# ToddThomson/Mila

Measured on AMD Instinct MI355X. Metric: Gemma-4 12B decode tok/s (B=1, context 2048), 1xMI355X, higher is better.
Workload: dtype bf16; 1 GPU; Gemma-4 12B, weight policy bf16, B=1, prefill T=2048 then decode at positions 2048..; decode_mode=graph, replicas=1, parallelism=replicas only (no collective), bounded_local_kv=0

## Files before the change

mila_amd/csrc/matvec.hip:

```cpp
#include <cstdio>
#include <cstdlib>

#include "common.h"
#include "internal.h"
#include "rms_common.h"
#include "matvec_body.h"

namespace mila {

struct MatvecTail
{
    void* y;
    const float* scales;
    const uint16_t* bias;
    const uint16_t* post_w;
    uint16_t* res_out;
    float post_scale, eps;
    int group, comb_splits, comb_heads;
    float* amax_v;
    int* amax_i;
};
static MatvecTail matvec_tail(const MatvecParams& p)
{
    return MatvecTail{p.y, p.scales, p.bias, p.post_w, p.res_out, p.post_scale, p.eps, p.group, p.comb_splits, p.comb_heads, p.amax_v, p.amax_i};
}

template <int FMT, int R, int U, int PRO, bool GEGLU, bool F32OUT, int XC, int XSRC = X_PLAIN>
__global__ __launch_bounds__(1024) void matvec_kernel(const uint8_t* W, const uint16_t* x, const uint16_t* norm_w, const uint16_t* res, int K, int N, int nblocks,
                                                      const MatvecTail t)
{
    extern __shared__ __attribute__((aligned(16))) unsigned char smem_raw[];
    __shared__ float red_a[16 * XC], red_b[16 * XC];
    u32x4 rkeep[XC];
    const MatvecParams p{t.y, x, W, t.scales, t.bias, norm_w, t.post_w, res, t.res_out, t.post_scale, t.eps, K, N, t.group, t.comb_splits, t.comb_heads, t.amax_v, t.amax_i};
    matvec_body<FMT, R, U, PRO, GEGLU, F32OUT ? Y_F32 : Y_BF16, XC, XSRC, RES_MEM>(
        p, reinterpret_cast<u32x4*>(smem_raw), red_a, red_b, (int)blockIdx.x, nblocks, rkeep, NoWait{});
}

static int g_tune_R = 0, g_tune_U = 0, g_tune_blocks = 0;
MILA_TUNE("matvec.rows_per_wave", g_tune_R);
MILA_TUNE("matvec.chunks_in_flight", g_tune_U);
MILA_TUNE("matvec.max_workgroups", g_tune_blocks);
static thread_local int t_last_matvec_blocks = 0;

template <int FMT, int R, int U, int PRO, bool GEGLU, bool F32OUT, int XC>
static int launch_xc(const MatvecParams& p, int max_blocks, hipStream_t s)
{
    const int n_rg = (p.N + R - 1) / R;
    constexpr int EPC = Fmt<FMT>::kElemsPerChunk;
    const int nchunks = p.K / EPC;
    const int S = (nchunks + 64 * U - 1) / (64 * U);
    const size_t lds = (size_t)S * 64 * U * EPC * 2;
    MILA_REQUIRE(lds <= 65536, "matvec: K=%d needs %zu bytes of LDS for x (limit 65536)", p.K, lds);
    int blocks = (n_rg + kMatvecWaves - 1) / kMatvecWaves;
    if (blocks > max_blocks) blocks = max_blocks;
    if (blocks < 1) blocks = 1;
    t_last_matvec_blocks = blocks;
    note_form("matvec");
    hipLaunchKernelGGL((matvec_kernel<FMT, R, U, PRO, GEGLU, F32OUT, XC>), dim3(blocks), dim3(64 * kMatvecWaves), lds, s, p.W, p.x, p.norm_w, p.res, p.K, p.N, blocks,
                       matvec_tail(p));
    MILA_LAUNCH_CHECK("matvec");
}

template <int FMT, int R, int U, int PRO, bool GEGLU, bool F32OUT>
static int launch(const MatvecParams& p, int max_blocks, hipStream_t s)
{
    if (p.K <= 8192) return launch_xc<FMT, R, U, PRO, GEGLU, F32OUT, 1>(p, max_blocks, s);
    if (p.K <= 16384) return launch_xc<FMT, R, U, PRO, GEGLU, F32OUT, 2>(p, max_blocks, s);
    return set_error(MILA_E_INVALID_ARGUMENT, "matvec: K=%d exceeds the register-staged x limit (16384)", p.K);
}

struct ShapeOverrides
{
    struct E { bool set = false; int rows = 1, U = 2, blocks = kNumCU; } e[3][3];
};
static ShapeOverrides parse_shape_overrides()
{
    ShapeOverrides o;
    const char* env = getenv("MILA_MATVEC_SHAPE");
    if (!env) return o;
    int f, t, r, u, b, n = 0;
    while (*env && sscanf(env, "f%dt%d=%d,%d,%d%n", &f, &t, &r, &u, &b, &n) == 5)
    {
        if (f >= 0 && f < 3 && t >= 0 && t < 3 && r >= 1 && u >= 1 && b >= 1) { o.e[f][t].set = true; o.e[f][t].rows = r; o.e[f][t].U = u; o.e[f][t].blocks = b; }
        env += n;
        if (*env == ';') ++env;
    }
    return o;
}

MatvecShape matvec_launch_shape(int fmt, bool geglu, int N, bool argmax)
{
    const int rows = geglu ? 2 * N : N;
    const bool tall = rows >= 16384, huge = rows >= 100000;
    int rows_per_step, U;
    if (fmt == FMT_BF16) { rows_per_step = huge ? 4 : (tall ? 2 : 1); U = tall ? 2 : 4; }
    else if (fmt == FMT_FP8) { rows_per_step = huge ? 4 : (tall ? 2 : 1); U = 2; }
    else { rows_per_step = tall ? 2 : 1; U = huge ? 2 : 1; }
    int max_blocks = (huge || (tall && fmt == FMT_BF16)) ? 2 * kNumCU : kNumCU;
    {
        static const ShapeOverrides ov = parse_shape_overrides();
        const ShapeOverrides::E& e = ov.e[fmt][huge ? 2 : (tall ? 1 : 0)];
        if (e.set) { rows_per_step = e.rows; U = e.U; max_blocks = e.blocks; }
    }
    int R = geglu ? (rows_per_step >= 2 ? rows_per_step / 2 : 1) : rows_per_step;
    if (g_tune_R > 0) R = g_tune_R;
    if (g_tune_U > 0) U = g_tune_U;
    if (g_tune_blocks > 0) max_blocks = g_tune_blocks;
    if (argmax && max_blocks > kArgmaxPartials) max_blocks = kArgmaxPartials;
    if (geglu && R > 2) R = 2;
    if (R == 1) U = (U == 1 || U == 2) ? U : 4;
    else if (R == 2) U = (U == 1) ? 1 : 2;
    else { R = geglu ? 2 : 4; U = 2; }
    return MatvecShape{R, U, max_blocks};
}

template <int FMT, int PRO, bool GEGLU, bool F32OUT>
static int dispatch_RU(const MatvecParams& p, hipStream_t s)
{
    const MatvecShape shape = matvec_launch_shape(FMT, GEGLU, p.N, p.amax_v != nullptr);
    const int R = shape.R, U = shape.U, max_blocks = shape.max_blocks;
    if (R == 1 && U == 1) return launch<FMT, 1, 1, PRO, GEGLU, F32OUT>(p, max_blocks, s);
    if (R == 1 && U == 2) return launch<FMT, 1, 2, PRO, GEGLU, F32OUT>(p, max_blocks, s);
    if (R == 1) return launch<FMT, 1, 4, PRO, GEGLU, F32OUT>(p, max_blocks, s);
    if (R == 2 && U == 1) return launch<FMT, 2, 1, PRO, GEGLU, F32OUT>(p, max_blocks, s);
    if (R == 2) return launch<FMT, 2, 2, PRO, GEGLU, F32OUT>(p, max_blocks, s);
    if constexpr (!GEGLU) return launch<FMT, 4, 2, PRO, GEGLU, F32OUT>(p, max_blocks, s);
    return launch<FMT, 2, 2, PRO, GEGLU, F32OUT>(p, max_blocks, s);
}

template <int FMT, int U, int XSRC>
static int launch_combine_t(const MatvecParams& p, hipStream_t s)
{
    constexpr int EPC = Fmt<FMT>::kElemsPerChunk;
    const int nchunks = p.K / EPC;
    const int S = (nchunks + 64 * U - 1) / (64 * U);
    const size_t lds = (size_t)S * 64 * U * EPC * 2;
    MILA_REQUIRE(lds <= 65536, "matvec_attn_combine: K=%d needs %zu bytes of LDS for x (limit 65536)", p.K, lds);
    int blocks = (p.N + kMatvecWaves - 1) / kMatvecWaves;
    if (blocks > kNumCU) blocks = kNumCU;
    hipLaunchKernelGGL((matvec_kernel<FMT, 1, U, 0, false, false, 1, XSRC>), dim3(blocks), dim3(64 * kMatvecWaves), lds, s, p.W, p.x, p.norm_w, p.res, p.K, p.N, blocks,
                       matvec_tail(p));
    MILA_LAUNCH_CHECK("matvec_attn_combine");
}
template <int XSRC>
static int launch_combine(int fmt, const MatvecParams& p, hipStream_t s)
{
    switch (fmt)
    {
        case FMT_BF16: return launch_combine_t<FMT_BF16, 4, XSRC>(p, s);
        case FMT_FP8: return launch_combine_t<FMT_FP8, 2, XSRC>(p, s);
        default: return launch_combine_t<FMT_FP4, 1, XSRC>(p, s);
    }
}

static int validate(const char* who, const void* y, const void* x, const void* W, const float* scales,
                    int fmt, int K, int N, int group)
{
    MILA_REQUIRE(y && x && W, "%s: null pointer (y=%p x=%p W=%p)", who, y, x, W);
    MILA_REQUIRE(K > 0 && N > 0, "%s: K and N must be positive (K=%d N=%d)", who, K, N);
    MILA_REQUIRE(K <= 16384, "%s: K=%d exceeds the register-staged x limit (16384)", who, K);
    if (fmt == FMT_BF16) MILA_REQUIRE(K % 8 == 0, "%s: K=%d must be a multiple of 8 for bf16 weights", who, K);
    if (fmt == FMT_FP8)
    {
        MILA_REQUIRE(K % 16 == 0, "%s: K=%d must be a multiple of 16 for fp8 weights", who, K);
        MILA_REQUIRE(scales != nullptr, "%s: fp8 weights need per-channel scales", who);
    }
    if (fmt == FMT_FP4)
    {
        MILA_REQUIRE(group == 64 || group == 128, "%s: fp4 group size must be 64 or 128 (got %d)", who, group);
        MILA_REQUIRE(K % 32 == 0 && K % group == 0, "%s: K=%d must be a multiple of 32 and of the group size %d", who, K, group);
        MILA_REQUIRE(scales != nullptr, "%s: fp4 weights need per-group scales", who);
    }
    MILA_REQUIRE(fmt >= 0 && fmt <= 2, "%s: unknown weight format %d", who, fmt);
    return MILA_OK;
}

template <int PRO, bool GEGLU, bool F32OUT>
static int dispatch_fmt(int fmt, const MatvecParams& p, hipStream_t s)
{
    switch (fmt)
    {
        case FMT_BF16: return dispatch_RU<FMT_BF16, PRO, GEGLU, F32OUT>(p, s);
        case FMT_FP8: return dispatch_RU<FMT_FP8, PRO, GEGLU, F32OUT>(p, s);
        default: return dispatch_RU<FMT_FP4, PRO, GEGLU, F32OUT>(p, s);
    }
}

}

using namespace mila;

extern "C" {

int mila_cdna4_matvec_bf16(uint16_t* y, const uint16_t* x, const uint16_t* W, const uint16_t* bias, int K,
                           int N, mila_stream_t stream)
{
    int rc = validate("matvec_bf16", y, x, W, nullptr, FMT_BF16, K, N, 0);
    if (rc) return rc;
    MatvecParams p{y, x, reinterpret_cast<const uint8_t*>(W), nullptr, bias, nullptr, nullptr, nullptr, nullptr, 1.0f, 0.0f, K, N, 0, 0, 0};
    return dispatch_fmt<0, false, false>(FMT_BF16, p, as_stream(stream));
}

int mila_cdna4_matvec_bf16_qfp8(uint16_t* y, const uint16_t* x, const uint8_t* W, const float* scales,
                                const uint16_t* bias, int K, int N, mila_stream_t stream)
{
    int rc = validate("matvec_bf16_qfp8", y, x, W, scales, FMT_FP8, K, N, 0);
    if (rc) return rc;
    MatvecParams p{y, x, W, scales, bias, nullptr, nullptr, nullptr, nullptr, 1.0f, 0.0f, K, N, 0, 0, 0};
    return dispatch_fmt<0, false, false>(FMT_FP8, p, as_stream(stream));
}

int mila_cdna4_matvec_bf16_qfp4(uint16_t* y, const uint16_t* x, const uint8_t* W_packed, const float* scales,
                                const uint16_t* bias, int K, int N, int group, mila_stream_t stream)
{
    int rc = validate("matvec_bf16_qfp4", y, x, W_packed, scales, FMT_FP4, K, N, group);
    if (rc) return rc;
    MatvecParams p{y, x, W_packed, scales, bias, nullptr, nullptr, nullptr, nullptr, 1.0f, 0.0f, K, N, group, 0, 0};
    return dispatch_fmt<0, false, false>(FMT_FP4, p, as_stream(stream));
}

int mila_cdna4_matvec_f32out(float* y, const uint16_t* x, const void* W, const float* scales, int fmt, int K,
                             int N, int group, mila_stream_t stream)
{
    int rc = validate("matvec_f32out", y, x, W, scales, fmt, K, N, group);
    if (rc) return rc;
    MatvecParams p{y, x, reinterpret_cast<const uint8_t*>(W), scales, nullptr, nullptr, nullptr, nullptr, nullptr, 1.0f, 0.0f, K, N, group, 0, 0};
    return dispatch_fmt<0, false, true>(fmt, p, as_stream(stream));
}

int mila_cdna4_matvec_attn_combine(uint16_t* y, const void* partials, int splits, int NH, int HS, const void* W, const float* scales,
                                   int fmt, int N, int group, mila_stream_t stream)
{
    MILA_REQUIRE(partials != nullptr, "matvec_attn_combine: null partials");
    MILA_REQUIRE(HS == 256 || HS == 512, "matvec_attn_combine: head size %d must be 256 or 512 (a wave's 64 chunks span 2 or 1 heads)", HS);
    MILA_REQUIRE(NH > 0 && splits > 1 && splits <= 64, "matvec_attn_combine: need NH > 0 and 1 < splits <= 64 (NH=%d splits=%d)", NH, splits);
    const int K = NH * HS;
    MILA_REQUIRE(K <= 8192, "matvec_attn_combine: NH * HS = %d exceeds 8192", K);
    int rc = validate("matvec_attn_combine", y, partials, W, scales, fmt, K, N, group);
    if (rc) return rc;
    MatvecParams p{y, reinterpret_cast<const uint16_t*>(partials), reinterpret_cast<const uint8_t*>(W), scales, nullptr, nullptr, nullptr, nullptr,
                   nullptr, 1.0f, 0.0f, K, N, group, splits, NH};
    return HS == 512 ? launch_combine<X_COMBINE_1>(fmt, p, as_stream(stream)) : launch_combine<X_COMBINE_2>(fmt, p, as_stream(stream));
}

int mila_cdna4_fused_norm_matvec(const mila_fused_matvec_args* a, mila_stream_t stream)
{
    MILA_REQUIRE(a != nullptr, "fused_norm_matvec: null args");
    const int rows = a->geglu ? 2 * a->N : a->N;
    (void)rows;
    int rc = validate("fused_norm_matvec", a->y, a->x, a->W, a->scales, a->fmt, a->K, a->N, a->group);
    if (rc) return rc;
    MILA_REQUIRE(a->norm_w != nullptr, "fused_norm_matvec: norm_w is required");
    MILA_REQUIRE((a->res == nullptr) == (a->post_w == nullptr), "fused_norm_matvec: res and post_w go together");
    if (a->res)
    {
        MILA_REQUIRE(a->res_out != nullptr, "fused_norm_matvec: res_out is required with res");
        MILA_REQUIRE(a->res_out != a->res && a->res_out != a->x, "fused_norm_matvec: res_out must not alias res or x");
    }
    MatvecParams p{a->y, a->x, reinterpret_cast<const uint8_t*>(a->W), a->scales, nullptr, a->norm_w, a->post_w,
                   a->res, a->res_out, a->post_scale, a->eps, a->K, a->N, a->group, 0, 0};
    hipStream_t s = as_stream(stream);
    MILA_REQUIRE(!(a->geglu && a->f32_out), "fused_norm_matvec: geglu and f32_out are exclusive");
    if (a->argmax_scratch)
    {
        MILA_REQUIRE(a->f32_out, "fused_norm_matvec: argmax_scratch needs f32_out (the logits)");
        MILA_REQUIRE(a->argmax_blocks != nullptr, "fused_norm_matvec: argmax_blocks is required with argmax_scratch");
        if (a->argmax_scratch_bytes < mila_cdna4_sample_scratch_bytes())
            return set_error(MILA_E_SCRATCH_TOO_SMALL, "fused_norm_matvec: argmax scratch %zu bytes < required %zu", a->argmax_scratch_bytes, mila_cdna4_sample_scratch_bytes());
        p.amax_v = reinterpret_cast<float*>(a->argmax_scratch);
        p.amax_i = reinterpret_cast<int*>(p.amax_v + kArgmaxPartials);
    }
    if (a->f32_out)
    {
        rc = a->res ? dispatch_fmt<2, false, true>(a->fmt, p, s) : dispatch_fmt<1, false, true>(a->fmt, p, s);
        if (rc == MILA_OK && a->argmax_scratch)
        {
            if (t_last_matvec_blocks > kArgmaxPartials) return set_error(MILA_E_RUNTIME, "fused_norm_matvec: %d workgroups exceed the %d sampler partials", t_last_matvec_blocks, kArgmaxPartials);
            *a->argmax_blocks = t_last_matvec_blocks;
        }
        return rc;
    }
    if (a->res)
        return a->geglu ? dispatch_fmt<2, true, false>(a->fmt, p, s) : dispatch_fmt<2, false, false>(a->fmt, p, s);
    return a->geglu ? dispatch_fmt<1, true, false>(a->fmt, p, s) : dispatch_fmt<1, false, false>(a->fmt, p, s);
}

}
```

mila_amd/csrc/matvec_body.h:

```cpp
#pragma once
#include "common.h"
#include "rms_common.h"

namespace mila {

enum { FMT_BF16 = 0, FMT_FP8 = 1, FMT_FP4 = 2 };

template <int FMT> struct Fmt;
template <> struct Fmt<FMT_BF16> { static constexpr int kElemsPerChunk = 8; };
template <> struct Fmt<FMT_FP8> { static constexpr int kElemsPerChunk = 16; };
template <> struct Fmt<FMT_FP4> { static constexpr int kElemsPerChunk = 32; };

template <int FMT>
__device__ __forceinline__ float chunk_dot(const u32x4 w, const u32x4* __restrict__ xs, int c, float acc)
{
    if constexpr (FMT == FMT_BF16)
    {
        const u32x4 xv = xs[c];
#pragma unroll
        for (int d = 0; d < 4; ++d) acc = dot2_bf16(as_bf16x2(w[d]), as_bf16x2(xv[d]), acc);
    }
    else if constexpr (FMT == FMT_FP8)
    {
        const u32x4 x0 = xs[2 * c], x1 = xs[2 * c + 1];
        acc = dot2_bf16(fp8x2_to_bf16x2(w[0], false), as_bf16x2(x0[0]), acc);
        acc = dot2_bf16(fp8x2_to_bf16x2(w[0], true), as_bf16x2(x0[1]), acc);
        acc = dot2_bf16(fp8x2_to_bf16x2(w[1], false), as_bf16x2(x0[2]), acc);
        acc = dot2_bf16(fp8x2_to_bf16x2(w[1], true), as_bf16x2(x0[3]), acc);
        acc = dot2_bf16(fp8x2_to_bf16x2(w[2], false), as_bf16x2(x1[0]), acc);
        acc = dot2_bf16(fp8x2_to_bf16x2(w[2], true), as_bf16x2(x1[1]), acc);
        acc = dot2_bf16(fp8x2_to_bf16x2(w[3], false), as_bf16x2(x1[2]), acc);
        acc = dot2_bf16(fp8x2_to_bf16x2(w[3], true), as_bf16x2(x1[3]), acc);
    }
    else
    {
#pragma unroll
        for (int d = 0; d < 4; ++d)
        {
            const u32x4 xv = xs[4 * c + d];
            acc = dot2_bf16(fp4x2_to_bf16x2<0>(w[d]), as_bf16x2(xv[0]), acc);
            acc = dot2_bf16(fp4x2_to_bf16x2<1>(w[d]), as_bf16x2(xv[1]), acc);
            acc = dot2_bf16(fp4x2_to_bf16x2<2>(w[d]), as_bf16x2(xv[2]), acc);
            acc = dot2_bf16(fp4x2_to_bf16x2<3>(w[d]), as_bf16x2(xv[3]), acc);
        }
    }
    return acc;
}

struct MatvecParams
{
    void* y;
    const uint16_t* x;
    const uint8_t* W;
    const float* scales;
    const uint16_t* bias;
    const uint16_t* norm_w;
    const uint16_t* post_w;
    const uint16_t* res;
    uint16_t* res_out;
    float post_scale, eps;
    int K, N, group;
    int comb_splits, comb_heads;
    float* amax_v = nullptr;
    int* amax_i = nullptr;
};

constexpr int kMatvecWaves = 16;

struct MatvecShape { int R, U, max_blocks; };
MatvecShape matvec_launch_shape(int fmt, bool geglu, int N, bool argmax);

template <int FMT, int U, int NR>
struct WBuf
{
    u32x4 w[U][NR];
    float sc[U][NR];
};

__device__ __forceinline__ uint32_t sload32(const void* p_uniform)
{
    uint32_t v;
    asm volatile("s_load_dword %0, %1, 0x0\n\ts_waitcnt lgkmcnt(0)" : "=s"(v) : "s"(p_uniform) : "memory");
    return v;
}

typedef __attribute__((address_space(1))) uint32_t gu32;
typedef __attribute__((address_space(1))) unsigned long long gu64;
__device__ __forceinline__ gu32* as_global(uint32_t* p) { return (gu32*)p; }
__device__ __forceinline__ const gu32* as_global(const uint32_t* p) { return (const gu32*)p; }
__device__ __forceinline__ gu64* as_global(unsigned long long* p) { return (gu64*)p; }
__device__ __forceinline__ const gu64* as_global(const unsigned long long* p) { return (const gu64*)p; }
__device__ __forceinline__ void handoff_store(uint32_t* v, int i, uint32_t bf16_bits)
{
    __hip_atomic_store(as_global(v) + i, bf16_bits, __ATOMIC_RELAXED, __HIP_MEMORY_SCOPE_AGENT);
}
__device__ __forceinline__ u32x4 handoff_load8(const uint32_t* v, int c)
{
    const gu64* q = as_global(reinterpret_cast<const unsigned long long*>(v)) + (size_t)c * 4;
    u32x4 r;
#pragma unroll
    for (int d = 0; d < 4; ++d)
    {
        const unsigned long long t = __hip_atomic_load(q + d, __ATOMIC_RELAXED, __HIP_MEMORY_SCOPE_AGENT);
        r[d] = ((uint32_t)t & 0xffffu) | ((uint32_t)(t >> 32) << 16);
    }
    return r;
}

struct NoWait { __device__ __forceinline__ void operator()() const {} };

enum { Y_BF16 = 0, Y_F32 = 1, Y_HANDOFF = 2 };
enum { X_PLAIN = 0, X_HANDOFF = 1, X_COMBINE_1 = 2, X_COMBINE_2 = 3 };
enum { RES_MEM = 0, RES_REG = 1 };

template <int FMT, int R, int U, int PRO, bool GEGLU, int YDST, int XC, int XSRC, int RSRC, class Wait>
__device__ __forceinline__ void matvec_body(const MatvecParams& p, u32x4* xs, float* red_a, float* red_b,
                                            const int block, const int nblocks, u32x4 (&rkeep)[XC], Wait wait)
{
    const int tid = threadIdx.x, lane = tid & 63;
    const int wib = __builtin_amdgcn_readfirstlane(tid >> 6);
    const int K = p.K, N = p.N;
    const int nx16 = K / 8;

    constexpr int EPC = Fmt<FMT>::kElemsPerChunk;
    constexpr int XPC = EPC / 8;
    constexpr int NR = GEGLU ? 2 * R : R;
    const int nchunks = K / EPC;
    const size_t row_bytes = (size_t)nchunks * 16;
    const int S = (nchunks + 64 * U - 1) / (64 * U);
    const int nx16_pad = S * 64 * U * XPC;
    const int ngroups = (FMT == FMT_FP4) ? K / p.group : 0;
    const int cpg_shift = (FMT == FMT_FP4) ? (p.group == 128 ? 2 : 1) : 0;
    const int total_waves = nblocks * kMatvecWaves;
    const int n_rg = (N + R - 1) / R;
    const int wave_g = block * kMatvecWaves + wib;
    const int nrg_w = wave_g < n_rg ? (n_rg - 1 - wave_g) / total_waves + 1 : 0;
    const int T = nrg_w * S;

    u32x4 px[XC], pnw[PRO != 0 ? XC : 1], ppw[PRO == 2 ? XC : 1], pres[PRO == 2 ? XC : 1];
#pragma unroll
    for (int k = 0; k < XC; ++k)
    {
        const size_t e = (size_t)min(tid + 1024 * k, nx16 - 1) * 8;
        if constexpr (XSRC == X_PLAIN) px[k] = ld16(p.x + e);
        if constexpr (PRO != 0) pnw[k] = ld16(p.norm_w + e);
        if constexpr (PRO == 2)
        {
            ppw[k] = ld16(p.post_w + e);
            if constexpr (RSRC == RES_MEM) pres[k] = ld16(p.res + e);
            else pres[k] = rkeep[k];
        }
    }

    auto issue = [&](WBuf<FMT, U, NR>& b, int rg, int s) {
        const int c0 = s * (64 * U) + lane;
#pragma unroll
        for (int j = 0; j < NR; ++j)
        {
            const int col = min(rg * R + (GEGLU ? (j >> 1) : j), N - 1);
            const int row = (GEGLU && (j & 1)) ? (N + col) : col;
            const uint8_t* wrow = p.W + (size_t)row * row_bytes;
#pragma unroll
            for (int u = 0; u < U; ++u)
            {
                const int c = min(c0 + 64 * u, nchunks - 1);
                b.w[u][j] = ld16_nt(wrow + (size_t)c * 16);
                if constexpr (FMT == FMT_FP4) b.sc[u][j] = p.scales[(size_t)row * ngroups + (c >> cpg_shift)];
            }
        }
    };
    int ci_rg = wave_g, ci_s = 0, cc_rg = wave_g, cc_s = 0;
    auto advance = [&](int& rg_, int& s_) {
        const bool wrap = (s_ + 1 == S);
        s_ = wrap ? 0 : s_ + 1;
        rg_ = wrap ? rg_ + total_waves : rg_;
    };
    WBuf<FMT, U, NR> ba, bb;
    issue(ba, ci_rg, ci_s); advance(ci_rg, ci_s);
    issue(bb, ci_rg, ci_s); advance(ci_rg, ci_s);

    if constexpr (XSRC == X_COMBINE_1 || XSRC == X_COMBINE_2)
    {
        constexpr int HPW = (XSRC == X_COMBINE_1) ? 1 : 2;
        const float* part = reinterpret_cast<const float*>(p.x);
        const int splits = p.comb_splits, HS = 512 / HPW, STR = HS + 4;
#pragma unroll
        for (int k = 0; k < XC; ++k)
        {
            const int c = tid + 1024 * k;
            const int h0 = ((c & ~63) * 8) / HS;
            const int myj = (HPW == 1) ? 0 : (lane >> 5);
            float fs[HPW], Lh[HPW];
#pragma unroll
            for (int j = 0; j < HPW; ++j)
            {
                const int h = min(h0 + j, p.comb_heads - 1);
                const float* hb = part + (size_t)h * splits * STR;
                const float ms = (lane < splits) ? hb[(size_t)lane * STR + HS] : -INFINITY;
                const float ls = (lane < splits) ? hb[(size_t)lane * STR + HS + 1] : 0.0f;
                const float M = wave_max(ms);
                fs[j] = (ms == -INFINITY) ? 0.0f : __expf(ms - M);
                Lh[j] = wave_sum(ls * fs[j]);
            }
            const int h = min(h0 + myj, p.comb_heads - 1);
            const float* vb = part + (size_t)h * splits * STR + (size_t)((c * 8) % HS);
            float acc[8];
#pragma unroll
            for (int e = 0; e < 8; ++e) acc[e] = 0.0f;
            for (int s0 = 0; s0 < splits; s0 += 8)
            {
                f32x4 va[8], vb2[8];
#pragma unroll
                for (int u = 0; u < 8; ++u)
                {
                    const float* src = vb + (size_t)min(s0 + u, splits - 1) * STR;
                    va[u] = *reinterpret_cast<const f32x4*>(src);
                    vb2[u] = *reinterpret_cast<const f32x4*>(src + 4);
                }
#pragma unroll
                for (int u = 0; u < 8; ++u)
                {
                    const int si = min(s0 + u, 63);
                    float f = __uint_as_float(__builtin_amdgcn_readlane(__float_as_uint(fs[0]), si));
                    if constexpr (HPW == 2)
                    {
                        const float f1 = __uint_as_float(__builtin_amdgcn_readlane(__float_as_uint(fs[1]), si));
                        f = myj ? f1 : f;
                    }
                    if (s0 + u >= splits) f = 0.0f;
#pragma unroll
                    for (int e = 0; e < 4; ++e)
                    {
                        acc[e] = fmaf(va[u][e], f, acc[e]);
                        acc[4 + e] = fmaf(vb2[u][e], f, acc[4 + e]);
                    }
                }
            }
            float L = Lh[0];
            if constexpr (HPW == 2) L = myj ? Lh[1] : Lh[0];
#pragma unroll
            for (int d = 0; d < 4; ++d)
                px[k][d] = pack_bf16x2(L > 0.0f ? acc[2 * d] / L : 0.0f, L > 0.0f ? acc[2 * d + 1] / L : 0.0f);
        }
    }

    wait();
    if constexpr (XSRC == X_HANDOFF)
    {
#pragma unroll
        for (int k = 0; k < XC; ++k)
            px[k] = handoff_load8(reinterpret_cast<const uint32_t*>(p.x), min(tid + 1024 * k, nx16 - 1));
    }

    for (int i = nx16 + tid; i < nx16_pad; i += 1024) xs[i] = u32x4{0u, 0u, 0u, 0u};
    if constexpr (PRO == 0)
    {
#pragma unroll
        for (int k = 0; k < XC; ++k)
            if (tid + 1024 * k < nx16) xs[tid + 1024 * k] = px[k];
    }
    else
    {
        const int G = (nx16 + 63) / 64;
        auto rstd_of = [&](const u32x4* v, float* red) {
#pragma unroll
            for (int k = 0; k < XC; ++k)
            {
                float s = (tid + 1024 * k < nx16) ? sumsq8(v[k], 0.0f) : 0.0f;
                s = wave_sum(s);
                if (lane == 0) red[wib + kMatvecWaves * k] = s;
            }
            __syncthreads();
            float t = 0.0f;
            for (int g = 0; g < G; ++g) t += red[g];
            return rsqrtf(t / (float)K + p.eps);
        };
        if constexpr (PRO == 1)
        {
            const float rstd = rstd_of(px, red_a);
#pragma unroll
            for (int k = 0; k < XC; ++k)
                if (tid + 1024 * k < nx16) xs[tid + 1024 * k] = rms_apply8(px[k], pnw[k], rstd, 0.0f);
        }
        else
        {
            const float rstd_a = rstd_of(px, red_a);
#pragma unroll
            for (int k = 0; k < XC; ++k) rkeep[k] = sandwich_tail8(rms_apply8(px[k], ppw[k], rstd_a, 0.0f), pres[k], p.post_scale);
            if (block == 0 && p.res_out != nullptr)
            {
#pragma unroll
                for (int k = 0; k < XC; ++k)
                    if (tid + 1024 * k < nx16) st16(p.res_out + (size_t)(tid + 1024 * k) * 8, rkeep[k]);
            }
            const float rstd_r = rstd_of(rkeep, red_b);
#pragma unroll
            for (int k = 0; k < XC; ++k)
                if (tid + 1024 * k < nx16) xs[tid + 1024 * k] = rms_apply8(rkeep[k], pnw[k], rstd_r, 0.0f);
        }
    }
    __syncthreads();

    float acc[NR];
#pragma unroll
    for (int j = 0; j < NR; ++j) acc[j] = 0.0f;

    auto compute = [&](const WBuf<FMT, U, NR>& b, int s) {
#pragma unroll
        for (int u = 0; u < U; ++u)
        {
            const int c = s * (64 * U) + lane + 64 * u;
#pragma unroll
            for (int j = 0; j < NR; ++j)
            {
                if constexpr (FMT == FMT_FP4)
                    acc[j] = fmaf(b.sc[u][j], chunk_dot<FMT>(b.w[u][j], xs, c, 0.0f), acc[j]);
                else
                    acc[j] = chunk_dot<FMT>(b.w[u][j], xs, c, acc[j]);
            }
        }
    };

    float amax_bv = -3.402823466e+38f;
    int amax_bi = 0x7fffffff;
    auto finish = [&](int rg_) {
        const int col0 = rg_ * R;
#pragma unroll
        for (int j = 0; j < NR; ++j) acc[j] = wave_sum(acc[j]);
#pragma unroll
        for (int j = 0; j < NR; ++j)
        {
            const int col = min(col0 + (GEGLU ? (j >> 1) : j), N - 1);
            const int row = (GEGLU && (j & 1)) ? (N + col) : col;
            float v = acc[j];
            if constexpr (FMT == FMT_FP8) v = __builtin_bit_cast(float, sload32(p.scales + row)) * v;
            if (p.bias)
            {
                const uint32_t pair = sload32(reinterpret_cast<const uint32_t*>(p.bias) + (row >> 1));
                v += bf16_bits_to_f32((uint16_t)((row & 1) ? (pair >> 16) : (pair & 0xffffu)));
            }
            acc[j] = v;
        }
        if (lane == 0)
        {
#pragma unroll
            for (int r = 0; r < R; ++r)
            {
                const int col = col0 + r;
                if (col >= N) continue;
                float v = acc[r];
                if constexpr (GEGLU)
                {
                    const float g = round_bf16(acc[2 * r]), up = round_bf16(acc[2 * r + 1]);
                    v = gelu_tanh(g) * up;
                }
                if constexpr (YDST == Y_F32)
                {
                    reinterpret_cast<float*>(p.y)[col] = v;
                    if (p.amax_v) argmax_better(amax_bv, amax_bi, v, col);
                }
                else if constexpr (YDST == Y_HANDOFF) handoff_store(reinterpret_cast<uint32_t*>(p.y), col, f32_to_bf16_bits(v));
                else reinterpret_cast<uint16_t*>(p.y)[col] = f32_to_bf16_bits(v);
            }
        }
#pragma unroll
        for (int j = 0; j < NR; ++j) acc[j] = 0.0f;
    };

    auto consume = [&](const WBuf<FMT, U, NR>& b) {
        compute(b, cc_s);
        const int rg_prev = cc_rg;
        advance(cc_rg, cc_s);
        if (cc_rg != rg_prev) finish(rg_prev);
    };

    int t = 0;
    for (; t + 4 <= T; t += 2)
    {
        consume(ba);
        issue(ba, ci_rg, ci_s); advance(ci_rg, ci_s);
        consume(bb);
        issue(bb, ci_rg, ci_s); advance(ci_rg, ci_s);
    }
    const int rem = T - t;
    if (rem >= 1)
    {
        consume(ba);
        if (rem == 3) issue(ba, ci_rg, ci_s);
    }
    if (rem >= 2) consume(bb);
    if (rem == 3) consume(ba);

    if constexpr (YDST == Y_F32)
    {
        if (p.amax_v)
        {
            __syncthreads();
            if (lane == 0) { red_a[wib] = amax_bv; red_b[wib] = __int_as_float(amax_bi); }
            __syncthreads();
            if (tid == 0)
            {
                float bv = red_a[0];
                int bi = __float_as_int(red_b[0]);
#pragma unroll
                for (int w = 1; w < kMatvecWaves; ++w) argmax_better(bv, bi, red_a[w], __float_as_int(red_b[w]));
                p.amax_v[block] = bv;
                p.amax_i[block] = bi;
            }
        }
    }
}

}
```

mila_amd/csrc/matvec_rows.hip:

```cpp
#include <cstdio>

#include "common.h"
#include "internal.h"
#include "rms_common.h"
#include "matvec_body.h"

namespace mila {

constexpr int kMaxMatvecRows = 4;
constexpr size_t kMatvecRowsLdsLimit = 160 * 1024;

struct MatvecRowsTail
{
    void* y;
    const float* scales;
    const uint16_t* bias;
    const uint16_t* post_w;
    uint16_t* res_out;
    float post_scale, eps;
    int group;
    long long x_stride, y_stride, res_stride, res_out_stride;
    float* amax_v;
    long long amax_stride;
};

template <int FMT, int U, int PRO, bool GEGLU, bool F32OUT, int XC, int NB>
__global__ __launch_bounds__(1024) void matvec_rows_kernel(const uint8_t* W, const uint16_t* x, const uint16_t* norm_w, const uint16_t* res, int K, int N, int nblocks,
                                                           const MatvecRowsTail t)
{
    extern __shared__ __attribute__((aligned(16))) unsigned char smem_raw[];
    __shared__ float red[NB][2][16 * XC];
    u32x4* xs0 = reinterpret_cast<u32x4*>(smem_raw);

    const int tid = threadIdx.x, lane = tid & 63;
    const int wib = __builtin_amdgcn_readfirstlane(tid >> 6);
    const int block = (int)blockIdx.x;
    const int nx16 = K / 8;

    constexpr int EPC = Fmt<FMT>::kElemsPerChunk;
    constexpr int XPC = EPC / 8;
    constexpr int NR = GEGLU ? 2 : 1;
    const int nchunks = K / EPC;
    const size_t row_bytes = (size_t)nchunks * 16;
    const int S = (nchunks + 64 * U - 1) / (64 * U);
    const int nx16_pad = S * 64 * U * XPC;
    const int ngroups = (FMT == FMT_FP4) ? K / t.group : 0;
    const int cpg_shift = (FMT == FMT_FP4) ? (t.group == 128 ? 2 : 1) : 0;
    const int total_waves = nblocks * kMatvecWaves;
    const int wave_g = block * kMatvecWaves + wib;
    const int ncol_w = wave_g < N ? (N - 1 - wave_g) / total_waves + 1 : 0;
    const int T = ncol_w * S;

    u32x4 px[NB][XC], pnw[PRO != 0 ? XC : 1], ppw[PRO == 2 ? XC : 1], pres[PRO == 2 ? NB : 1][XC];
#pragma unroll
    for (int k = 0; k < XC; ++k)
    {
        const size_t e = (size_t)min(tid + 1024 * k, nx16 - 1) * 8;
#pragma unroll
        for (int b = 0; b < NB; ++b)
        {
            px[b][k] = ld16(x + (size_t)b * t.x_stride + e);
            if constexpr (PRO == 2) pres[b][k] = ld16(res + (size_t)b * t.res_stride + e);
        }
        if constexpr (PRO != 0) pnw[k] = ld16(norm_w + e);
        if constexpr (PRO == 2) ppw[k] = ld16(t.post_w + e);
    }

    auto issue = [&](WBuf<FMT, U, NR>& wb, int col_, int s) {
        const int c0 = s * (64 * U) + lane;
        const int col = min(col_, N - 1);
#pragma unroll
        for (int j = 0; j < NR; ++j)
        {
            const int row = j ? (N + col) : col;
            const uint8_t* wrow = W + (size_t)row * row_bytes;
#pragma unroll
            for (int u = 0; u < U; ++u)
            {
                const int c = min(c0 + 64 * u, nchunks - 1);
                wb.w[u][j] = ld16_nt(wrow + (size_t)c * 16);
                if constexpr (FMT == FMT_FP4) wb.sc[u][j] = t.scales[(size_t)row * ngroups + (c >> cpg_shift)];
            }
        }
    };
    int ci_col = wave_g, ci_s = 0, cc_col = wave_g, cc_s = 0;
    auto advance = [&](int& col_, int& s_) {
        const bool wrap = (s_ + 1 == S);
        s_ = wrap ? 0 : s_ + 1;
        col_ = wrap ? col_ + total_waves : col_;
    };
    WBuf<FMT, U, NR> ba, bb;
    issue(ba, ci_col, ci_s); advance(ci_col, ci_s);
    issue(bb, ci_col, ci_s); advance(ci_col, ci_s);

#pragma unroll
    for (int b = 0; b < NB; ++b)
        for (int i = nx16 + tid; i < nx16_pad; i += 1024) xs0[(size_t)b * nx16_pad + i] = u32x4{0u, 0u, 0u, 0u};
    if constexpr (PRO == 0)
    {
#pragma unroll
        for (int b = 0; b < NB; ++b)
#pragma unroll
            for (int k = 0; k < XC; ++k)
                if (tid + 1024 * k < nx16) xs0[(size_t)b * nx16_pad + tid + 1024 * k] = px[b][k];
    }
    else
    {
        const int G = (nx16 + 63) / 64;
        auto rstd_of = [&](const u32x4* v, float* r) {
#pragma unroll
            for (int k = 0; k < XC; ++k)
            {
                float s = (tid + 1024 * k < nx16) ? sumsq8(v[k], 0.0f) : 0.0f;
                s = wave_sum(s);
                if (lane == 0) r[wib + kMatvecWaves * k] = s;
            }
            __syncthreads();
            float tt = 0.0f;
            for (int g = 0; g < G; ++g) tt += r[g];
            return rsqrtf(tt / (float)K + t.eps);
        };
#pragma unroll
        for (int b = 0; b < NB; ++b)
        {
            u32x4* xs = xs0 + (size_t)b * nx16_pad;
            if constexpr (PRO == 1)
            {
                const float rstd = rstd_of(px[b], red[b][0]);
#pragma unroll
                for (int k = 0; k < XC; ++k)
                    if (tid + 1024 * k < nx16) xs[tid + 1024 * k] = rms_apply8(px[b][k], pnw[k], rstd, 0.0f);
            }
            else
            {
                u32x4 rk[XC];
                const float rstd_a = rstd_of(px[b], red[b][0]);
#pragma unroll
                for (int k = 0; k < XC; ++k) rk[k] = sandwich_tail8(rms_apply8(px[b][k], ppw[k], rstd_a, 0.0f), pres[b][k], t.post_scale);
                if (block == 0 && t.res_out != nullptr)
                {
#pragma unroll
                    for (int k = 0; k < XC; ++k)
                        if (tid + 1024 * k < nx16) st16(t.res_out + (size_t)b * t.res_out_stride + (size_t)(tid + 1024 * k) * 8, rk[k]);
                }
                const float rstd_r = rstd_of(rk, red[b][1]);
#pragma unroll
                for (int k = 0; k < XC; ++k)
                    if (tid + 1024 * k < nx16) xs[tid + 1024 * k] = rms_apply8(rk[k], pnw[k], rstd_r, 0.0f);
            }
        }
    }
    __syncthreads();

    float acc[NB][NR];
#pragma unroll
    for (int b = 0; b < NB; ++b)
#pragma unroll
        for (int j = 0; j < NR; ++j) acc[b][j] = 0.0f;

    auto compute = [&](const WBuf<FMT, U, NR>& wb, int s) {
#pragma unroll
        for (int u = 0; u < U; ++u)
        {
            const int c = s * (64 * U) + lane + 64 * u;
#pragma unroll
            for (int j = 0; j < NR; ++j)
#pragma unroll
                for (int b = 0; b < NB; ++b)
                {
                    const u32x4* xs = xs0 + (size_t)b * nx16_pad;
                    if constexpr (FMT == FMT_FP4)
                        acc[b][j] = fmaf(wb.sc[u][j], chunk_dot<FMT>(wb.w[u][j], xs, c, 0.0f), acc[b][j]);
                    else
                        acc[b][j] = chunk_dot<FMT>(wb.w[u][j], xs, c, acc[b][j]);
                }
        }
    };

    float amax_bv[NB];
    int amax_bi[NB];
#pragma unroll
    for (int b = 0; b < NB; ++b) { amax_bv[b] = -3.402823466e+38f; amax_bi[b] = 0x7fffffff; }

    auto finish = [&](int col) {
        float scale[NR], bias[NR];
#pragma unroll
        for (int j = 0; j < NR; ++j)
        {
            const int row = j ? (N + col) : col;
            scale[j] = 1.0f;
            bias[j] = 0.0f;
            if constexpr (FMT == FMT_FP8) scale[j] = __builtin_bit_cast(float, sload32(t.scales + row));
            if (t.bias)
            {
                const uint32_t pair = sload32(reinterpret_cast<const uint32_t*>(t.bias) + (row >> 1));
                bias[j] = bf16_bits_to_f32((uint16_t)((row & 1) ? (pair >> 16) : (pair & 0xffffu)));
            }
        }
#pragma unroll
        for (int b = 0; b < NB; ++b)
        {
#pragma unroll
            for (int j = 0; j < NR; ++j)
            {
                float v = wave_sum(acc[b][j]);
                if constexpr (FMT == FMT_FP8) v = scale[j] * v;
                if (t.bias) v += bias[j];
                acc[b][j] = v;
            }
            if (lane == 0)
            {
                float v = acc[b][0];
                if constexpr (GEGLU)
                {
                    const float g = round_bf16(acc[b][0]), up = round_bf16(acc[b][1]);
                    v = gelu_tanh(g) * up;
                }
                if constexpr (F32OUT)
                {
                    reinterpret_cast<float*>(t.y)[(size_t)b * t.y_stride + col] = v;
                    if (t.amax_v) argmax_better(amax_bv[b], amax_bi[b], v, col);
                }
                else reinterpret_cast<uint16_t*>(t.y)[(size_t)b * t.y_stride + col] = f32_to_bf16_bits(v);
            }
#pragma unroll
            for (int j = 0; j < NR; ++j) acc[b][j] = 0.0f;
        }
    };

    auto consume = [&](const WBuf<FMT, U, NR>& wb) {
        compute(wb, cc_s);
        const int col_prev = cc_col;
        advance(cc_col, cc_s);
        if (cc_col != col_prev) finish(col_prev);
    };

    int ts = 0;
    for (; ts + 4 <= T; ts += 2)
    {
        consume(ba);
        issue(ba, ci_col, ci_s); advance(ci_col, ci_s);
        consume(bb);
        issue(bb, ci_col, ci_s); advance(ci_col, ci_s);
    }
    const int rem = T - ts;
    if (rem >= 1)
    {
        consume(ba);
        if (rem == 3) issue(ba, ci_col, ci_s);
    }
    if (rem >= 2) consume(bb);
    if (rem == 3) consume(ba);

    if constexpr (F32OUT)
    {
        if (t.amax_v)
        {
            __syncthreads();
            if (lane == 0)
            {
#pragma unroll
                for (int b = 0; b < NB; ++b) { red[b][0][wib] = amax_bv[b]; red[b][1][wib] = __int_as_float(amax_bi[b]); }
            }
            __syncthreads();
            if (tid < NB)
            {
                float bv = red[tid][0][0];
                int bi = __float_as_int(red[tid][1][0]);
                for (int w = 1; w < kMatvecWaves; ++w) argmax_better(bv, bi, red[tid][0][w], __float_as_int(red[tid][1][w]));
                float* pv = t.amax_v + (size_t)tid * t.amax_stride;
                pv[block] = bv;
                reinterpret_cast<int*>(pv + kArgmaxPartials)[block] = bi;
            }
        }
    }
}

struct MatvecRowsArgs
{
    const uint8_t* W;
    const uint16_t* x;
    const uint16_t* norm_w;
    const uint16_t* res;
    int K, N;
    MatvecRowsTail t;
};

struct MatvecRowsPlan { int R, U, xc; size_t lds, lds_static; int blocks; };

static bool plan_rows(int fmt, int K, int N, bool geglu, bool argmax, int rows, MatvecRowsPlan& pl)
{
    if (fmt < 0 || fmt > 2 || K <= 0 || N <= 0 || K > 16384 || rows < 1 || rows > kMaxMatvecRows) return false;
    const int epc = fmt == FMT_BF16 ? 8 : (fmt == FMT_FP8 ? 16 : 32);
    if (K % epc != 0) return false;
    const MatvecShape shape = matvec_launch_shape(fmt, geglu, N, argmax);
    pl.R = rows == 1 ? shape.R : 1;
    pl.U = shape.U;
    pl.xc = K <= 8192 ? 1 : 2;
    const int nchunks = K / epc;
    const int S = (nchunks + 64 * pl.U - 1) / (64 * pl.U);
    pl.lds = (size_t)rows * S * 64 * pl.U * epc * 2;
    pl.lds_static = rows > 1 ? (size_t)rows * 2 * 16 * pl.xc * sizeof(float) : (size_t)2 * 16 * pl.xc * sizeof(float);
    const int n_rg = (N + pl.R - 1) / pl.R;
    int blocks = (n_rg + kMatvecWaves - 1) / kMatvecWaves;
    if (blocks > shape.max_blocks) blocks = shape.max_blocks;
    pl.blocks = blocks < 1 ? 1 : blocks;
    return true;
}

template <int FMT, int U, int PRO, bool GEGLU, bool F32OUT, int XC, int NB>
static int launch_rows_t(const MatvecRowsArgs& a, const MatvecRowsPlan& pl, hipStream_t s)
{
    auto kernel = matvec_rows_kernel<FMT, U, PRO, GEGLU, F32OUT, XC, NB>;
    static thread_local int raised_for = -1;
    int dev = 0;
    if (pl.lds > 65536)
    {
        int rc = check_hip(hipGetDevice(&dev), "matvec_rows");
        if (rc) return rc;
        if (raised_for != dev)
        {
            rc = check_hip(hipFuncSetAttribute(reinterpret_cast<const void*>(kernel), hipFuncAttributeMaxDynamicSharedMemorySize, (int)kMatvecRowsLdsLimit), "matvec_rows");
            if (rc) return rc;
            raised_for = dev;
        }
    }
    note_form("matvec_rows");
    hipLaunchKernelGGL(kernel, dim3(pl.blocks), dim3(64 * kMatvecWaves), pl.lds, s, a.W, a.x, a.norm_w, a.res, a.K, a.N, pl.blocks, a.t);
    MILA_LAUNCH_CHECK("matvec_rows");
}

template <int FMT, int U, int PRO, bool GEGLU, bool F32OUT, int XC>
static int launch_rows_nb(const MatvecRowsArgs& a, const MatvecRowsPlan& pl, int rows, hipStream_t s)
{
    if (rows == 2) return launch_rows_t<FMT, U, PRO, GEGLU, F32OUT, XC, 2>(a, pl, s);
    if (rows == 3) return launch_rows_t<FMT, U, PRO, GEGLU, F32OUT, XC, 3>(a, pl, s);
    return launch_rows_t<FMT, U, PRO, GEGLU, F32OUT, XC, 4>(a, pl, s);
}

template <int FMT, int PRO, bool GEGLU, bool F32OUT>
static int launch_rows_u(const MatvecRowsArgs& a, const MatvecRowsPlan& pl, int rows, hipStream_t s)
{
    if (pl.xc == 1)
    {
        if (pl.U == 1) return launch_rows_nb<FMT, 1, PRO, GEGLU, F32OUT, 1>(a, pl, rows, s);
        if (pl.U == 2) return launch_rows_nb<FMT, 2, PRO, GEGLU, F32OUT, 1>(a, pl, rows, s);
        return launch_rows_nb<FMT, 4, PRO, GEGLU, F32OUT, 1>(a, pl, rows, s);
    }
    if (pl.U == 1) return launch_rows_nb<FMT, 1, PRO, GEGLU, F32OUT, 2>(a, pl, rows, s);
    if (pl.U == 2) return launch_rows_nb<FMT, 2, PRO, GEGLU, F32OUT, 2>(a, pl, rows, s);
    return launch_rows_nb<FMT, 4, PRO, GEGLU, F32OUT, 2>(a, pl, rows, s);
}

template <int PRO, bool GEGLU, bool F32OUT>
static int launch_rows_fmt(int fmt, const MatvecRowsArgs& a, const MatvecRowsPlan& pl, int rows, hipStream_t s)
{
    switch (fmt)
    {
        case FMT_BF16: return launch_rows_u<FMT_BF16, PRO, GEGLU, F32OUT>(a, pl, rows, s);
        case FMT_FP8: return launch_rows_u<FMT_FP8, PRO, GEGLU, F32OUT>(a, pl, rows, s);
        default: return launch_rows_u<FMT_FP4, PRO, GEGLU, F32OUT>(a, pl, rows, s);
    }
}

}

using namespace mila;

extern "C" {

size_t mila_cdna4_matvec_rows_plan_describe(int fmt, int K, int N, int geglu, int f32_out, int rows, char* buf, size_t cap)
{
    if (buf && cap) buf[0] = 0;
    MatvecRowsPlan pl;
    if ((geglu && f32_out) || !plan_rows(fmt, K, N, geglu != 0, f32_out != 0, rows, pl) || pl.lds + pl.lds_static > kMatvecRowsLdsLimit) return 0;
    return 1 + snprintf(buf, buf ? cap : 0, "%d:%d:%d:%zu:%d", pl.R, pl.U, pl.xc, pl.lds, pl.blocks);
}

int mila_cdna4_matvec_rows(const mila_matvec_rows_args* r, mila_stream_t stream)
{
    MILA_REQUIRE(r != nullptr, "matvec_rows: null args");
    const mila_fused_matvec_args* a = &r->a;
    MILA_REQUIRE(a->y && a->x && a->W, "matvec_rows: null pointer (y=%p x=%p W=%p)", (const void*)a->y, (const void*)a->x, a->W);
    MILA_REQUIRE(a->K > 0 && a->N > 0, "matvec_rows: K and N must be positive (K=%d N=%d)", a->K, a->N);
    MILA_REQUIRE(a->fmt >= 0 && a->fmt <= 2, "matvec_rows: unknown weight format %d", a->fmt);
    MILA_REQUIRE(a->K <= 16384, "matvec_rows: K=%d exceeds the register-staged x limit (16384)", a->K);
    if (a->fmt == FMT_BF16) MILA_REQUIRE(a->K % 8 == 0, "matvec_rows: K=%d must be a multiple of 8 for bf16 weights", a->K);
    if (a->fmt == FMT_FP8)
    {
        MILA_REQUIRE(a->K % 16 == 0, "matvec_rows: K=%d must be a multiple of 16 for fp8 weights", a->K);
        MILA_REQUIRE(a->scales != nullptr, "matvec_rows: fp8 weights need per-channel scales");
    }
    if (a->fmt == FMT_FP4)
    {
        MILA_REQUIRE(a->group == 64 || a->group == 128, "matvec_rows: fp4 group size must be 64 or 128 (got %d)", a->group);
        MILA_REQUIRE(a->K % 32 == 0 && a->K % a->group == 0, "matvec_rows: K=%d must be a multiple of 32 and of the group size %d", a->K, a->group);
        MILA_REQUIRE(a->scales != nullptr, "matvec_rows: fp4 weights need per-group scales");
    }
    if (r->rows < 2 || r->rows > kMaxMatvecRows)
        return set_error(MILA_E_UNSUPPORTED, "matvec_rows: rows=%d is outside 2 .. %d (one row: the matvec_* / fused_norm_matvec entries)", r->rows, kMaxMatvecRows);
    const int rows = r->rows;
    const bool geglu = a->geglu != 0, f32 = a->f32_out != 0;
    MILA_REQUIRE(!(geglu && f32), "matvec_rows: geglu and f32_out are exclusive");
    MILA_REQUIRE(a->norm_w != nullptr || (!a->res && !a->post_w && !geglu), "matvec_rows: res / post_w / geglu need norm_w (the fused forms)");
    MILA_REQUIRE(a->norm_w == nullptr || r->bias == nullptr, "matvec_rows: bias goes with the plain form (norm_w == NULL) only");
    MILA_REQUIRE(!(f32 && r->bias), "matvec_rows: bias goes with bf16 output only (matvec_f32out takes none: no one-row entry defines those bits)");
    MILA_REQUIRE((a->res == nullptr) == (a->post_w == nullptr), "matvec_rows: res and post_w go together");
    const long long out_w = a->N;
    MILA_REQUIRE(r->x_stride >= a->K && r->y_stride >= out_w, "matvec_rows: x_stride %lld / y_stride %lld below the row widths %d / %lld", (long long)r->x_stride,
                 (long long)r->y_stride, a->K, out_w);
    if (a->res)
    {
        MILA_REQUIRE(a->res_out != nullptr, "matvec_rows: res_out is required with res");
        MILA_REQUIRE(a->res_out != a->res && a->res_out != a->x, "matvec_rows: res_out must not alias res or x");
        MILA_REQUIRE(r->res_stride >= a->K && r->res_out_stride >= a->K, "matvec_rows: res_stride %lld / res_out_stride %lld below the row width %d", (long long)r->res_stride,
                     (long long)r->res_out_stride, a->K);
    }
    MILA_REQUIRE(r->x_stride % 8 == 0 && (!a->res || (r->res_stride % 8 == 0 && r->res_out_stride % 8 == 0)), "matvec_rows: x / res / res_out row strides must be multiples of 8 elements (16-byte accesses)");

    MatvecRowsPlan pl;
    if (!plan_rows(a->fmt, a->K, a->N, geglu, a->argmax_scratch != nullptr, rows, pl)) return set_error(MILA_E_INVALID_ARGUMENT, "matvec_rows: no plan for fmt=%d K=%d N=%d", a->fmt, a->K, a->N);
    if (pl.lds + pl.lds_static > kMatvecRowsLdsLimit)
        return set_error(MILA_E_UNSUPPORTED, "matvec_rows: K=%d at %d rows needs %zu bytes of LDS for x (limit %zu)", a->K, rows, pl.lds, kMatvecRowsLdsLimit);

    MatvecRowsArgs k{reinterpret_cast<const uint8_t*>(a->W), a->x, a->norm_w, a->res, a->K, a->N,
                     MatvecRowsTail{a->y, a->scales, r->bias, a->post_w, a->res_out, a->norm_w ? a->post_scale : 1.0f, a->eps, a->group, r->x_stride, r->y_stride,
                                    r->res_stride, r->res_out_stride, nullptr, 0}};
    if (a->argmax_scratch)
    {
        MILA_REQUIRE(f32, "matvec_rows: argmax_scratch needs f32_out (the logits)");
        MILA_REQUIRE(a->argmax_blocks != nullptr, "matvec_rows: argmax_blocks is required with argmax_scratch");
        const size_t per_row = mila_cdna4_sample_scratch_bytes();
        if (a->argmax_scratch_bytes < per_row * rows)
            return set_error(MILA_E_SCRATCH_TOO_SMALL, "matvec_rows: argmax scratch %zu bytes < required %zu (%d rows)", a->argmax_scratch_bytes, per_row * rows, rows);
        if (pl.blocks > kArgmaxPartials) return set_error(MILA_E_RUNTIME, "matvec_rows: %d workgroups exceed the %d sampler partials", pl.blocks, kArgmaxPartials);
        k.t.amax_v = reinterpret_cast<float*>(a->argmax_scratch);
        k.t.amax_stride = (long long)(per_row / sizeof(float));
    }
    hipStream_t s = as_stream(stream);
    int rc;
    if (!a->norm_w) rc = f32 ? launch_rows_fmt<0, false, true>(a->fmt, k, pl, rows, s) : launch_rows_fmt<0, false, false>(a->fmt, k, pl, rows, s);
    else if (f32) rc = a->res ? launch_rows_fmt<2, false, true>(a->fmt, k, pl, rows, s) : launch_rows_fmt<1, false, true>(a->fmt, k, pl, rows, s);
    else if (a->res) rc = geglu ? launch_rows_fmt<2, true, false>(a->fmt, k, pl, rows, s) : launch_rows_fmt<2, false, false>(a->fmt, k, pl, rows, s);
    else rc = geglu ? launch_rows_fmt<1, true, false>(a->fmt, k, pl, rows, s) : launch_rows_fmt<1, false, false>(a->fmt, k, pl, rows, s);
    if (rc == MILA_OK && a->argmax_scratch) *a->argmax_blocks = pl.blocks;
    return rc;
}

}
```

Baseline: 228.0 tok/s.

## Add lean matvec variants for two-workgroups-per-CU occupancy and defer second weight prefetch

```diff
diff --git a/mila_amd/csrc/matvec.hip b/mila_amd/csrc/matvec.hip
--- a/mila_amd/csrc/matvec.hip
+++ b/mila_amd/csrc/matvec.hip
@@ -25,15 +25,20 @@
     return MatvecTail{p.y, p.scales, p.bias, p.post_w, p.res_out, p.post_scale, p.eps, p.group, p.comb_splits, p.comb_heads, p.amax_v, p.amax_i};
 }
 
+template <int FMT, int R, int U, bool GEGLU, int XC, int XSRC>
+constexpr bool kTwoPerCU = XC == 1 && XSRC == X_PLAIN && FMT != FMT_FP4 && U == 2 && R == (GEGLU ? 1 : 2);
+template <int FMT, int R, int U, bool GEGLU, int XC, int XSRC>
+constexpr bool kLean = kTwoPerCU<FMT, R, U, GEGLU, XC, XSRC> || (XC == 1 && XSRC == X_PLAIN && FMT == FMT_BF16 && R == 1 && U == 4 && !GEGLU);
+
 template <int FMT, int R, int U, int PRO, bool GEGLU, bool F32OUT, int XC, int XSRC = X_PLAIN>
-__global__ __launch_bounds__(1024) void matvec_kernel(const uint8_t* W, const uint16_t* x, const uint16_t* norm_w, const uint16_t* res, int K, int N, int nblocks,
+__global__ __launch_bounds__(1024, (kLean<FMT, R, U, GEGLU, XC, XSRC> ? 8 : 0)) void matvec_kernel(const uint8_t* W, const uint16_t* x, const uint16_t* norm_w, const uint16_t* res, int K, int N, int nblocks,
                                                       const MatvecTail t)
 {
     extern __shared__ __attribute__((aligned(16))) unsigned char smem_raw[];
     __shared__ float red_a[16 * XC], red_b[16 * XC];
     u32x4 rkeep[XC];
     const MatvecParams p{t.y, x, W, t.scales, t.bias, norm_w, t.post_w, res, t.res_out, t.post_scale, t.eps, K, N, t.group, t.comb_splits, t.comb_heads, t.amax_v, t.amax_i};
-    matvec_body<FMT, R, U, PRO, GEGLU, F32OUT ? Y_F32 : Y_BF16, XC, XSRC, RES_MEM>(
+    matvec_body<FMT, R, U, PRO, GEGLU, F32OUT ? Y_F32 : Y_BF16, XC, XSRC, RES_MEM, kLean<FMT, R, U, GEGLU, XC, XSRC>>(
         p, reinterpret_cast<u32x4*>(smem_raw), red_a, red_b, (int)blockIdx.x, nblocks, rkeep, NoWait{});
 }
 
@@ -97,22 +102,24 @@
     if (fmt == FMT_BF16) { rows_per_step = huge ? 4 : (tall ? 2 : 1); U = tall ? 2 : 4; }
     else if (fmt == FMT_FP8) { rows_per_step = huge ? 4 : (tall ? 2 : 1); U = 2; }
     else { rows_per_step = tall ? 2 : 1; U = huge ? 2 : 1; }
-    int max_blocks = (huge || (tall && fmt == FMT_BF16)) ? 2 * kNumCU : kNumCU;
+    int max_blocks = (huge || (tall && fmt != FMT_FP4)) ? 2 * kNumCU : kNumCU;
+    int max_blocks_rows = (huge || (tall && fmt == FMT_BF16)) ? 2 * kNumCU : kNumCU;
     {
         static const ShapeOverrides ov = parse_shape_overrides();
         const ShapeOverrides::E& e = ov.e[fmt][huge ? 2 : (tall ? 1 : 0)];
-        if (e.set) { rows_per_step = e.rows; U = e.U; max_blocks = e.blocks; }
+        if (e.set) { rows_per_step = e.rows; U = e.U; max_blocks = max_blocks_rows = e.blocks; }
     }
     int R = geglu ? (rows_per_step >= 2 ? rows_per_step / 2 : 1) : rows_per_step;
     if (g_tune_R > 0) R = g_tune_R;
     if (g_tune_U > 0) U = g_tune_U;
-    if (g_tune_blocks > 0) max_blocks = g_tune_blocks;
+    if (g_tune_blocks > 0) max_blocks = max_blocks_rows = g_tune_blocks;
     if (argmax && max_blocks > kArgmaxPartials) max_blocks = kArgmaxPartials;
+    if (argmax && max_blocks_rows > kArgmaxPartials) max_blocks_rows = kArgmaxPartials;
     if (geglu && R > 2) R = 2;
     if (R == 1) U = (U == 1 || U == 2) ? U : 4;
     else if (R == 2) U = (U == 1) ? 1 : 2;
     else { R = geglu ? 2 : 4; U = 2; }
-    return MatvecShape{R, U, max_blocks};
+    return MatvecShape{R, U, max_blocks, max_blocks_rows};
 }
 
 template <int FMT, int PRO, bool GEGLU, bool F32OUT>
diff --git a/mila_amd/csrc/matvec_body.h b/mila_amd/csrc/matvec_body.h
--- a/mila_amd/csrc/matvec_body.h
+++ b/mila_amd/csrc/matvec_body.h
@@ -67,7 +67,7 @@
 
 constexpr int kMatvecWaves = 16;
 
-struct MatvecShape { int R, U, max_blocks; };
+struct MatvecShape { int R, U, max_blocks, max_blocks_rows; };
 MatvecShape matvec_launch_shape(int fmt, bool geglu, int N, bool argmax);
 
 template <int FMT, int U, int NR>
@@ -113,7 +113,7 @@
 enum { X_PLAIN = 0, X_HANDOFF = 1, X_COMBINE_1 = 2, X_COMBINE_2 = 3 };
 enum { RES_MEM = 0, RES_REG = 1 };
 
-template <int FMT, int R, int U, int PRO, bool GEGLU, int YDST, int XC, int XSRC, int RSRC, class Wait>
+template <int FMT, int R, int U, int PRO, bool GEGLU, int YDST, int XC, int XSRC, int RSRC, bool LEAN = false, class Wait>
 __device__ __forceinline__ void matvec_body(const MatvecParams& p, u32x4* xs, float* red_a, float* red_b,
                                             const int block, const int nblocks, u32x4 (&rkeep)[XC], Wait wait)
 {
@@ -164,7 +164,8 @@
             for (int u = 0; u < U; ++u)
             {
                 const int c = min(c0 + 64 * u, nchunks - 1);
-                b.w[u][j] = ld16_nt(wrow + (size_t)c * 16);
+                if constexpr (LEAN) b.w[u][j] = ld16_nt(wrow + (uint32_t)c * 16u);
+                else b.w[u][j] = ld16_nt(wrow + (size_t)c * 16);
                 if constexpr (FMT == FMT_FP4) b.sc[u][j] = p.scales[(size_t)row * ngroups + (c >> cpg_shift)];
             }
         }
@@ -176,8 +177,9 @@
         rg_ = wrap ? rg_ + total_waves : rg_;
     };
     WBuf<FMT, U, NR> ba, bb;
+    constexpr bool LATE_B = LEAN && PRO == 2 && XSRC == X_PLAIN;
     issue(ba, ci_rg, ci_s); advance(ci_rg, ci_s);
-    issue(bb, ci_rg, ci_s); advance(ci_rg, ci_s);
+    if constexpr (!LATE_B) { issue(bb, ci_rg, ci_s); advance(ci_rg, ci_s); }
 
     if constexpr (XSRC == X_COMBINE_1 || XSRC == X_COMBINE_2)
     {
@@ -272,7 +274,13 @@
             }
             __syncthreads();
             float t = 0.0f;
-            for (int g = 0; g < G; ++g) t += red[g];
+            if constexpr (LEAN)
+            {
+#pragma unroll 1
+                for (int g = 0; g < G; ++g) t += red[g];
+            }
+            else
+                for (int g = 0; g < G; ++g) t += red[g];
             return rsqrtf(t / (float)K + p.eps);
         };
         if constexpr (PRO == 1)
@@ -287,6 +295,7 @@
             const float rstd_a = rstd_of(px, red_a);
 #pragma unroll
             for (int k = 0; k < XC; ++k) rkeep[k] = sandwich_tail8(rms_apply8(px[k], ppw[k], rstd_a, 0.0f), pres[k], p.post_scale);
+            if constexpr (LATE_B) { issue(bb, ci_rg, ci_s); advance(ci_rg, ci_s); }
             if (block == 0 && p.res_out != nullptr)
             {
 #pragma unroll
diff --git a/mila_amd/csrc/matvec_rows.hip b/mila_amd/csrc/matvec_rows.hip
--- a/mila_amd/csrc/matvec_rows.hip
+++ b/mila_amd/csrc/matvec_rows.hip
@@ -303,7 +303,8 @@
     pl.lds_static = rows > 1 ? (size_t)rows * 2 * 16 * pl.xc * sizeof(float) : (size_t)2 * 16 * pl.xc * sizeof(float);
     const int n_rg = (N + pl.R - 1) / pl.R;
     int blocks = (n_rg + kMatvecWaves - 1) / kMatvecWaves;
-    if (blocks > shape.max_blocks) blocks = shape.max_blocks;
+    const int max_blocks = rows == 1 ? shape.max_blocks : shape.max_blocks_rows;
+    if (blocks > max_blocks) blocks = max_blocks;
     pl.blocks = blocks < 1 ? 1 : blocks;
     return true;
 }
```

New measurement: 230.0 tok/s (median of 6 runs). Within noise of the previous version (+0.9%).
